# nomadkaraoke/python-audio-separator

Measured on AMD Instinct MI355X. Metric: audio-sec separated / wall-sec (RTF), UVR-MDX-NET 44.1kHz stereo, 1/2/4/8 GPU, higher is better.
Workload: dtype f32 (I/O and accumulators; matrix products on the 16-bit pipe from block-scaled two-part fp16 operands, 22-bit products -- see arithmetic; fp32-exact setting timed in arithmetic_ab)

## Files before the change

python-audio-separator_amd/csrc/asx.hip:

```cpp
#include <hip/hip_runtime.h>

#include <algorithm>
#include <atomic>
#include <cmath>
#include <cstdarg>
#include <cstdio>
#include <cstdlib>
#include <cstring>
#include <functional>
#include <map>
#include <string>
#include <mutex>
#include <vector>

#include "../../include/asx.h"
#include "knobs.h"
#include "resample_plan.h"
#include "flac_dec_plan.h"

static void grant_lds(const void *kernel, int bytes) {
  static std::mutex mu;
  static std::map<const void *, int> granted;
  std::lock_guard<std::mutex> lock(mu);
  int &g = granted[kernel];
// ... 35 lines not shown
#include "engine_mdx.h"

static int opt_nonneg(int32_t v) { return v < 0 ? 0 : (int)v; }
static int opt_onoff(int32_t v) { return v > 0 ? 1 : 0; }

static const struct EngineOption {
  const char *key;
  int asx_engine::*field;
  int EngineKnobs::*knob;
  int (*norm)(int32_t);
  const char *refusal = nullptr;
  int shipped = 0;
} kOptions[] = {
    {"winograd", &asx_engine::winograd, &EngineKnobs::winograd, opt_nonneg,
     "asx_set_option: winograd = %d names a superseded kernel generation that only an experimental build carries "
     "(python build.py --experimental); this library has 0 (direct kernel) and 3 (the default)", 3},
    {"winograd_stationary", &asx_engine::winos, &EngineKnobs::winos, opt_nonneg,
     "asx_set_option: the weight-stationary Winograd kernel (measured slower) is in experimental builds only (python build.py --experimental)"},
    {"winograd_bf16x6", &asx_engine::wino6, &EngineKnobs::wino6, opt_nonneg},
    {"gemm_bf16x6", &asx_engine::gemm_bf16x6, &EngineKnobs::gemm_bf16x6, opt_onoff},
    {"gemm_f16x3", &asx_engine::gemm_f16x3, &EngineKnobs::gemm_f16x3, opt_onoff},
    {"conv_direct_f16x3", &asx_engine::conv3h, &EngineKnobs::conv3h, opt_nonneg},
    {"conv_fuse_input", &asx_engine::conv_fuse_input, &EngineKnobs::conv_fuse_input, opt_onoff},
    {"conv3h_partial_scratch", &asx_engine::conv3h_ps, &EngineKnobs::conv3h_ps, opt_onoff},
    {"conv3h_walk", &asx_engine::conv3h_walk, &EngineKnobs::conv3h_walk, opt_onoff},
    {"conv3h_tiled", &asx_engine::conv3h_tiled, &EngineKnobs::conv3h_tiled, opt_onoff},
    {"conv_down_bf16x6", &asx_engine::down6, &EngineKnobs::down6, opt_onoff},
    {"conv_up_bf16x6", &asx_engine::up6, &EngineKnobs::up6, opt_onoff},
    {"gemm_pair_images", &asx_engine::pair_images, &EngineKnobs::pair_images, opt_onoff,
     "asx_set_option: gemm_pair_images = 1 needs an experimental build (python build.py --experimental): the pair-image reader measured no "
     "faster in the nets and is not in the default library"},
};

static const EngineOption *find_option(const char *fn, const char *key) {
  for (const EngineOption &o : kOptions)
    if (!strcmp(key, o.key)) return &o;
  set_err("%s: unknown option '%s'", fn, key);
  return nullptr;
}

extern "C" {

int asx_abi_version(void) { return ASX_ABI_VERSION; }
const char *asx_last_error(void) { return g_err; }

int asx_device_count(void) {
// ... 115 lines not shown
  }
  *out = e;
  return ASX_OK;
}

static void v3_destroy(V3Net *n);
static void rof_destroy(RofNet *n);
static void ht_destroy(HtNet *n);
static void hd_destroy(HdNet *n);
static void hd_drop_clones(asx_engine *e);
static void vr_destroy(VrNet *n);
static void ens_destroy(EnsCtx *c);
static void free_conv(ConvLayer &L) {
  L.w.release();
  L.b.release();
  L.wu.release();
  L.wu2.release();
  L.wu3.release();
  L.wus.release();
  L.wu6.release();
  L.wu6h.release();
  L.w3h.release();
  L.w1f.release();
  L.wd6.release();
  L.wup6.release();
  L.gn_w.release();
  L.gn_b.release();
}
static void free_tdf(TdfLayer &L) {
  L.w.release();
  L.bias.release();
  L.scale.release();
  L.shift.release();
  L.gn_w.release();
  L.gn_b.release();
}
static void free_block(Block &b) {
  for (auto &c : b.tfc) free_conv(c);
  free_tdf(b.tdf0);
  free_tdf(b.tdf1);
}

void asx_engine_destroy(asx_engine *e) {
  w3_flush(e);
  if (!e) return;
  (void)hipSetDevice(e->device);
// ... 2461 lines not shown
  BufGuard g{{&dw, &dp, &ds}};
  CHK(to_dev(dw, wave_host, (size_t)2 * n_samples));
  if (primary_host) CHK(dp.ensure((size_t)2 * n_out * 4));
  if (secondary_host) CHK(ds.ensure((size_t)2 * n_out * 4));
  CHK(vr_separate_dev(e, dw.f(), n_samples, params, primary_host ? dp.f() : nullptr, secondary_host ? ds.f() : nullptr, nullptr));
  if (primary_host) CHK(to_host(primary_host, dp, (size_t)2 * n_out));
  if (secondary_host) CHK(to_host(secondary_host, ds, (size_t)2 * n_out));
  return ASX_OK;
}

int asx_counter(const asx_engine *e, const char *name, int64_t *out) {
  REQUIRE(e && name && out, "asx_counter: null argument");
  const std::string nm(name);
  if (nm == "tdf3_launches") *out = (int64_t)g_tdf3_launches.load();
  else if (nm == "tdf3h_launches") *out = (int64_t)g_tdf3h_launches.load();
  else if (nm == "attn6_launches") *out = (int64_t)g_attn6_launches.load();
  else if (nm == "attn6h_launches") *out = (int64_t)g_attn6h_launches.load();
  else if (nm == "tdf3_gather_launches") *out = (int64_t)g_tdf3_gather_launches.load();
  else if (nm == "wino6_launches") *out = (int64_t)g_wino6_launches.load();
  else if (nm == "wino6h_launches") *out = (int64_t)g_wino6h_launches.load();
  else if (nm == "conv3h_launches") *out = (int64_t)g_conv3h_launches.load();
  else if (nm == "conv3h_fin_launches") *out = (int64_t)g_conv3h_fin_launches.load();
  else if (nm == "conv3h_tiled_launches") *out = (int64_t)g_conv3h_tiled_launches.load();
  else if (nm == "tdf3_pair_image_launches") *out = (int64_t)g_tdf3ps_launches.load();
  else if (nm == "down6_launches") *out = (int64_t)g_down6_launches.load();
  else if (nm == "up6_launches") *out = (int64_t)g_up6_launches.load();
  else if (nm == "hd_rounds") *out = (int64_t)g_hd_rounds.load();
  else if (nm == "vr_net_passes") *out = (int64_t)g_vr_net_passes.load();
  else if (nm == "v3_net_passes") *out = (int64_t)g_v3_net_passes.load();
  else if (nm == "rof_net_passes") *out = (int64_t)g_rof_net_passes.load();
  else if (nm == "flac_block_cycles") *out = (int64_t)e->flac_block_cycles;
  else if (nm == "flac_crc16_cycles") *out = (int64_t)e->flac_crc16_cycles;
  else {
    set_err("asx_counter: unknown counter '%s'", name);
    return ASX_ERR_INVALID;
  }
  return ASX_OK;
}

int asx_debug_trace(uint64_t *host, int64_t n_u64) {
  REQUIRE(host && n_u64 > 0 && n_u64 <= 4096 * 8, "asx_debug_trace: bad argument");
  HIPCHK(hipDeviceSynchronize());
  HIPCHK(hipMemcpyFromSymbol(host, HIP_SYMBOL(asx_dbg_trace), (size_t)n_u64 * 8));
  return ASX_OK;
}

// ... 258 lines not shown
```

python-audio-separator_amd/csrc/engine_core.h:

```cpp
#pragma once

static thread_local char g_err[512] = "";
static void set_err(const char *fmt, ...) {
  va_list ap;
  va_start(ap, fmt);
  vsnprintf(g_err, sizeof(g_err), fmt, ap);
  va_end(ap);
}
#define HIPCHK(x)                                                                       \
  do {                                                                                  \
    hipError_t e_ = (x);                                                                \
    if (e_ != hipSuccess) {                                                             \
      set_err("%s:%d %s -> %s", __FILE__, __LINE__, #x, hipGetErrorString(e_));         \
      return ASX_ERR_HIP;                                                               \
    }                                                                                   \
  } while (0)
#define CHK(x)                    \
  do {                            \
    int r_ = (x);                 \
    if (r_ != ASX_OK) return r_;  \
  } while (0)
#define REQUIRE(cond, ...)        \
  do {                            \
    if (!(cond)) {                \
// ... 56 lines not shown
  return to_host(out_host, dout, n_out);
}

enum ConvKind { CK_3X3 = 0, CK_DOWN = 1, CK_1X1 = 2, CK_UP = 3 };

struct ConvLayer {
  int kind = CK_3X3;
  int cin = 0, cout = 0;
  int nrep = 0, kc = 0, cg = 0, nci = 0;
  int relu = 1;
  DevBuf w, b;
  DevBuf wu;
  DevBuf wu2;
  DevBuf wu3;
  int wu_cg = 0, wu_nci = 0, wu3_nci = 0;
  DevBuf wus;
  int wus_ks = 0;
  DevBuf gn_w, gn_b;
  DevBuf wu6;
  int wu6_nci = 0;
  DevBuf wu6h;
  DevBuf w3h;
  DevBuf w1f;
  DevBuf wd6;
  int wd6_cg = 0, wd6_nst = 0, wd6_nrep = 3;
  DevBuf wup6;
  int wup6_cg = 0, wup6_nst = 0;
};

struct TdfLayer {
  int n = 0, k = 0, c = 0;
  bool has_bias = false;
  DevBuf w, bias, scale, shift;
  DevBuf gn_w, gn_b;
};

struct Block {
  std::vector<ConvLayer> tfc;
  TdfLayer tdf0, tdf1;
  int c = 0, t = 0, f = 0;
};

struct ProfRec {
  int cls;
  int nprod;
  hipEvent_t a, b;
// ... 79 lines not shown
  DevBuf flac_cycles;
  long long flac_block_cycles = 0, flac_crc16_cycles = 0;
  DevBuf flac_frames, flac_off;
  DevBuf flacdec_list, flacdec_slots, flacdec_accept;
  std::vector<flacdec::Accept> flacdec_accept_host;
  int64_t flacdec_n_samples = -1, flacdec_n_frames = 0;
  int32_t flacdec_channels = 0, flacdec_bps = 0, flacdec_max_bs = 0;
  size_t flacdec_slot_off = 0;
  std::vector<RsTable *> rs_tabs;
  std::mutex rs_mu;
  hipEvent_t div_ev = nullptr;
  hipStream_t div_stream = nullptr;
  std::vector<DevBuf> skip;
  int winograd = 3;
  int winos = 0;
  int gemm_bf16x6 = 1;
  int gemm_f16x3 = 1;
  int wino6 = 144;
  int conv3h = 144;
  int conv3h_ps = 1;
  int conv3h_walk = 1;
  int conv3h_tiled = 1;
  int conv_fuse_input = 1;
  int down6 = 1;
  int up6 = 1;
  int pair_images = 0;
  std::vector<W3Entry> w3;
  std::mutex w3_mu;
  bool prof = false;
  int prof_nprod = 0;
  std::vector<ProfRec> recs;
};

static int pick_batch(const asx_engine *e) { return e->cfg.max_batch > 0 ? e->cfg.max_batch : 64; }

#include "batching.h"

template <class F>
static int timed(asx_engine *e, int cls, double flops, double bytes, hipStream_t s, F &&launch) {
  if (!e->prof) {
    launch();
    HIPCHK(hipGetLastError());
    return ASX_OK;
  }
  ProfRec r;
  r.cls = cls;
// ... 65 lines not shown
```

python-audio-separator_amd/csrc/engine_mdx.h:

```cpp
#pragma once

template <class CFG>
static void launch_conv_t(const ConvArgs &a, int nblk, hipStream_t s) {
  grant_lds(&conv_mfma_kernel<CFG>, CFG::LDS_BYTES);
  hipLaunchKernelGGL(conv_mfma_kernel<CFG>, dim3(nblk), dim3(256), CFG::LDS_BYTES, s, a);
}

static int conv_tile_h(int kind) { return kind == CK_UP ? 4 : 8; }

static int pick_nrep_conv(int cout) {
  const int ct = (cout + 15) / 16;
  int best = 1, best_pad = 1 << 30;
  for (int n = 3; n >= 1; --n) {
    const int pad = ((ct + n - 1) / n) * n - ct;
    if (pad < best_pad) {
      best_pad = pad;
      best = n;
    }
  }
  return best;
}
static int pick_nrep_up(int cout) {
  const int ct = (cout + 15) / 16;
  if (knobs().up_nrep == 4 && (4 * ct) % 4 == 0) return 4;
// ... 134 lines not shown
        for (int c = 0; c < L.cin; ++c) {
          const float *g = &w[((size_t)co * L.cin + c) * 9];
          double t[4][3];
          for (int a = 0; a < 4; ++a)
            for (int j = 0; j < 3; ++j) t[a][j] = G[a][0] * g[0 * 3 + j] + G[a][1] * g[1 * 3 + j] + G[a][2] * g[2 * 3 + j];
          float *dst = &wus[(size_t)(co / 48) * per];
          for (int a = 0; a < 4; ++a)
            for (int bb = 0; bb < 4; ++bb) {
              const float u = (float)(t[a][0] * G[bb][0] + t[a][1] * G[bb][1] + t[a][2] * G[bb][2]);
              dst[L.wus_ks == 12 ? winos_u_index<12>(a, bb, c, co % 48) : winos_u_index<24>(a, bb, c, co % 48)] = u;
            }
        }
      CHK(L.wus.ensure(wus.size() * 4));
      HIPCHK(hipMemcpy(L.wus.p, wus.data(), wus.size() * 4, hipMemcpyHostToDevice));
    }
#endif
  }
  if (L.kind == CK_1X1 && L.cin == 4 && L.cout == Conv3hCfg::C) {
    std::vector<float> w1((size_t)Conv3hCfg::C * 5, 0.f);
    memcpy(w1.data(), w, (size_t)Conv3hCfg::C * 4 * 4);
    if (b) memcpy(w1.data() + Conv3hCfg::C * 4, b, (size_t)Conv3hCfg::C * 4);
    CHK(L.w1f.ensure(w1.size() * 4));
    HIPCHK(hipMemcpy(L.w1f.p, w1.data(), w1.size() * 4, hipMemcpyHostToDevice));
  }
  if (L.kind == CK_DOWN) {
    std::vector<uint32_t> w6;
    L.wd6_nrep = (knobs().down6_wide && L.cout % 96 == 0) ? 6 : 3;
    if (L.wd6_nrep == 6) down6_pack<6>(w, L.cout, L.cin, w6, &L.wd6_cg, &L.wd6_nst);
    else down6_pack<3>(w, L.cout, L.cin, w6, &L.wd6_cg, &L.wd6_nst);
    CHK(L.wd6.ensure(w6.size() * 4));
    HIPCHK(hipMemcpy(L.wd6.p, w6.data(), w6.size() * 4, hipMemcpyHostToDevice));
  }
  if (L.kind == CK_UP) {
    std::vector<uint32_t> w6;
    if (L.nrep == 6) up6_pack<6>(w, L.cout, L.cin, w6, &L.wup6_cg, &L.wup6_nst);
    else if (L.nrep == 4) up6_pack<4>(w, L.cout, L.cin, w6, &L.wup6_cg, &L.wup6_nst);
    else up6_pack<2>(w, L.cout, L.cin, w6, &L.wup6_cg, &L.wup6_nst);
    CHK(L.wup6.ensure(w6.size() * 4));
    HIPCHK(hipMemcpy(L.wup6.p, w6.data(), w6.size() * 4, hipMemcpyHostToDevice));
  }
  const int nb = (L.kind == CK_UP) ? CT * 16 : std::max(L.cg * NW, ((L.cout + 47) / 48) * 48);
  std::vector<float> bp(nb, 0.f);
  for (int i = 0; i < L.cout; ++i) bp[i] = b ? b[i] : 0.f;
  CHK(L.w.ensure(wp.size() * 4));
  CHK(L.b.ensure(bp.size() * 4));
  HIPCHK(hipMemcpy(L.w.p, wp.data(), wp.size() * 4, hipMemcpyHostToDevice));
// ... 645 lines not shown
  }
#endif
  launch_tdf3_abl<NREP, MREP, 0>(a, w3, s);
  return true;
}

static int tdf3_tile_form(const asx_engine *e, const TdfDmaArgs &d) {
  const int t128 = knobs().gemm_t128;
  const int small = knobs().tdf2_small;
  if (!tdf3_ok(e, d) || d.N <= 64) return 0;
  if (d.N <= 128) return 1;
  if ((small && d.K <= small) || d.prefer_small) return 1;
  const double rows = (double)((d.M + 127) / 128);
  auto cost = [&](int bn, double eff) {
    const double blocks = rows * (double)((d.N + bn - 1) / bn);
    return ceil(blocks / 512.0) * bn / eff;
  };
  const double eff128 = knobs().tdf3_eff128;
  const double e128 = (e->gemm_f16x3 > 0 && d.K <= 512 && !knobs().tdf3_eff128_set) ? 1.0 : eff128;
  const bool narrow3 = t128 == 2 || (t128 == 1 && cost(128, e128) < cost(192, 1.0));
  return narrow3 ? 2 : 3;
}

static bool tdf3h_will_run(asx_engine *e, const TdfDmaArgs &d, hipStream_t s) {
  const bool dbg = knobs().tdf3_abl_set || knobs().f16x3_n_set;
  if (dbg || e->gemm_f16x3 <= 0 || e->pair_images <= 0 || tdf3_tile_form(e, d) == 0) return false;
  return w3_image(e, d.w, d.N, d.K, s, 0, 1) != nullptr;
}
static int tdf3_tile_cols(const asx_engine *e, const TdfDmaArgs &d) { return tdf3_tile_form(e, d) == 3 ? 192 : 128; }
static void tdf3_set_xexp(TdfDmaArgs &d, const int *tab, int cols) {
  d.xexp = tab;
  d.xexp_gs = cols / 32;
  d.xexp_n = (d.K + cols - 1) / cols;
  d.xexp_inv = (65536 + d.xexp_gs - 1) / d.xexp_gs;
}

static void launch_tdf_dma_auto(asx_engine *e, const TdfDmaArgs &d, hipStream_t s) {
  const int t128 = knobs().gemm_t128;
  const bool v2 = tdf2_ok(d);
  const int small = knobs().tdf2_small;
  const int form = tdf3_tile_form(e, d);
  if (form == 1 && d.N > 128 && launch_tdf3<2, 4>(e, d, s)) return;
  if (v2 && ((small && d.K <= small) || d.prefer_small) && d.N > 128) return launch_tdf2<2, 4>(d, s);
  if (d.N > 128) {
    const double rows = (double)((d.M + 127) / 128);
    auto cost = [&](int bn, double eff) {
      const double blocks = rows * (double)((d.N + bn - 1) / bn);
      return ceil(blocks / 512.0) * bn / eff;
    };
    const bool narrow = t128 == 2 || (t128 == 1 && cost(128, 0.96) < cost(192, 1.0));
    if (form == 2 && launch_tdf3<2, 8>(e, d, s)) return;
    if (form == 3 && launch_tdf3<3, 8>(e, d, s)) return;
    if (narrow) v2 ? launch_tdf2<2, 8>(d, s) : launch_tdf_dma_t<2, 8>(d, s);
    else v2 ? launch_tdf2<3, 8>(d, s) : launch_tdf_dma_t<3, 8>(d, s);
  } else if (d.N > 64) {
    if (form == 1 && launch_tdf3<2, 4>(e, d, s)) return;
    v2 ? launch_tdf2<2, 4>(d, s) : launch_tdf_dma_t<2, 4>(d, s);
// ... 45 lines not shown
  TdfDmaArgs d;
  tdf_fill_args(e, L, x, res, y, M, T, relu, d);
  if (pair_out) {
    d.yexp = pair_out;
    d.yexp_n = (L.n + pair_cols - 1) / pair_cols;
  }
  if (pair_in) tdf3_set_xexp(d, pair_in, pair_cols);
  if ((pair_out || pair_in) && !dma) {
    set_err("tdf_launch: pair image on a layer the row-GEMM kernels cannot take");
    return ASX_ERR_STATE;
  }
  return timed(e, ASX_PROF_TDF, flops, bytes, s, [&]() {
    if (dma) {
      launch_tdf_dma_auto(e, d, s);
    } else {
      if (L.n > 128) launch_tdf_t<3, 8>(a, s);
      else if (L.n > 64) launch_tdf_t<2, 4>(a, s);
      else launch_tdf_t<1, 4>(a, s);
    }
  });
}

static int tdf_pair_launch(asx_engine *e, const TdfLayer &L0, const TdfLayer &L1, const float *x, float *H, int *HE, float *out, int64_t M, int T,
                           hipStream_t s) {
  int *pair_tab = nullptr;
  int pair_cols = 0;
  if (M > 0 && HE != nullptr) {
    TdfDmaArgs d0, d1;
    tdf_fill_args(e, L0, x, nullptr, H, M, T, 1, d0);
    tdf_fill_args(e, L1, H, x, out, M, T, 1, d1);
    const bool al = ((reinterpret_cast<uintptr_t>(x) | reinterpret_cast<uintptr_t>(H)) & 15) == 0 && !knobs().no_dma;
    if (al && L0.n % 32 == 0 && L0.k % 4 == 0 && L1.k % 4 == 0 && tdf3h_will_run(e, d0, s) && tdf3h_will_run(e, d1, s)) {
      pair_cols = tdf3_tile_cols(e, d0);
      pair_tab = HE;
    }
  }
  CHK(tdf_launch(e, L0, x, nullptr, H, M, T, s, 1, pair_tab, nullptr, pair_cols));
  return tdf_launch(e, L1, H, x, out, M, T, s, 1, nullptr, pair_tab, pair_cols);
}

static int tdf_pack(TdfLayer &L, int n, int k, int c, const float *w, const float *bias, const float *scale,
                    const float *shift) {
  L.n = n;
  L.k = k;
  L.c = c;
  L.has_bias = bias != nullptr;
  CHK(L.w.ensure((size_t)n * k * 4));
  HIPCHK(hipMemcpy(L.w.p, w, (size_t)n * k * 4, hipMemcpyHostToDevice));
  if (bias) {
    CHK(L.bias.ensure((size_t)n * 4));
    HIPCHK(hipMemcpy(L.bias.p, bias, (size_t)n * 4, hipMemcpyHostToDevice));
  }
  if (scale && shift) {
    CHK(L.scale.ensure((size_t)c * 4));
    CHK(L.shift.ensure((size_t)c * 4));
    HIPCHK(hipMemcpy(L.scale.p, scale, (size_t)c * 4, hipMemcpyHostToDevice));
    HIPCHK(hipMemcpy(L.shift.p, shift, (size_t)c * 4, hipMemcpyHostToDevice));
  }
  return ASX_OK;
}
// ... 115 lines not shown
      else hipLaunchKernelGGL(f3::istft3p_kernel<0>, dim3(ng, 2, B), dim3(256), f3::ISTFT3P_LDS_BYTES, s, f);
    }
    else
      hipLaunchKernelGGL(f3::istft3_kernel, dim3(ng, 2, B), dim3(256), f3::ISTFT3_LDS_BYTES, s, f);
    if (ng > 1) hipLaunchKernelGGL(f3::seam3_kernel, dim3(5, ng - 1, B * 2), dim3(256), 0, s, f);
  });
}

static int gn_launch(asx_engine *e, const float *x, int B, int C, int64_t P, const DevBuf &gw, const DevBuf &gb, const float *res,
                     const float *mul, float *y, hipStream_t s) {
  if (B <= 0) return ASX_OK;
  REQUIRE(C % 2 == 0 && gw.p && gb.p && e->gn_part.bytes >= (size_t)B * C * 16, "GroupNorm(2, %d): channels / workspace", C);
  double2 *part = reinterpret_cast<double2 *>(e->gn_part.p);
  const double bytes = 4.0 * (double)B * C * (double)P;
  CHK(timed(e, ASX_PROF_MISC, 0.0, bytes, s,
            [&]() { hipLaunchKernelGGL(gn_partial_kernel, dim3((unsigned)C, (unsigned)B), dim3(256), 0, s, x, C, P, part); }));
  const int nx = (int)std::max<int64_t>(1, std::min<int64_t>(32, (P / 4 + 1023) / 1024));
  return timed(e, ASX_PROF_MISC, 0.0, bytes * (2 + (res ? 1 : 0) + (mul ? 1 : 0)), s, [&]() {
    hipLaunchKernelGGL(gn_apply_kernel, dim3((unsigned)nx, (unsigned)C, (unsigned)B), dim3(256), 0, s, x, C, 2, P, part, gw.f(), gb.f(), 1e-5f, 1, res,
                       mul, y);
  });
}

static int block_forward(asx_engine *e, const Block &blk, float *&cur, float *dest, int B, hipStream_t s, const float *fin_x = nullptr) {
  auto next_free = [&](const float *a, const float *b) -> float * {
    for (int i = 0; i < 3; ++i)
      if (e->R[i].f() != a && e->R[i].f() != b) return e->R[i].f();
    return nullptr;
  };
  const bool gn = e->net.norm == 1;
  const int64_t plane = (int64_t)blk.t * blk.f;
  auto c3h = [&](size_t j, const float *xin) {
    const ConvLayer &L = blk.tfc[j];
    const bool dma = blk.f % 4 == 0 && (reinterpret_cast<uintptr_t>(xin) & 15) == 0 && !knobs().no_dma;
    return conv3h_takes(e, L, dma, nullptr, L.relu ? ACT_RELU : ACT_NONE, blk.t, blk.f, (int64_t)L.cout * plane, e->R[0].f()) && conv3h_tiled_ok(e, L, blk.t);
  };
  bool in_tiled = false;
  for (size_t j = 0; j < blk.tfc.size(); ++j) {
    float *out = next_free(cur, nullptr);
    ConvView v;
    if (j == 0 && fin_x) {
      v.fin = &e->first;
      v.fin_x = fin_x;
    }
    v.x_tiled = in_tiled;
    v.y_tiled = e->conv3h_tiled > 0 && !gn && j + 1 < blk.tfc.size() && (in_tiled || c3h(j, j == 0 && fin_x ? fin_x : cur)) && c3h(j + 1, out);
    in_tiled = v.y_tiled;
// ... 13 lines not shown
  if (bnk == 0) {
    float *out = dest ? dest : next_free(cur, nullptr);
    if (gn) {
      float *tmp = next_free(cur, out);
      CHK(tdf_launch(e, blk.tdf0, cur, nullptr, tmp, M, blk.t, s, 0));
      CHK(gn_launch(e, tmp, B, blk.c, plane, blk.tdf0.gn_w, blk.tdf0.gn_b, cur, nullptr, out, s));
    } else {
      CHK(tdf_launch(e, blk.tdf0, cur, cur, out, M, blk.t, s));
    }
    cur = out;
    return ASX_OK;
  }
  if (gn) {
    CHK(tdf_launch(e, blk.tdf0, cur, nullptr, e->H.f(), M, blk.t, s, 0));
    CHK(gn_launch(e, e->H.f(), B, blk.c, (int64_t)blk.t * (blk.f / bnk), blk.tdf0.gn_w, blk.tdf0.gn_b, nullptr, nullptr, e->H.f(), s));
    float *out = dest ? dest : next_free(cur, nullptr);
    float *tmp = dest ? next_free(cur, nullptr) : out;
    CHK(tdf_launch(e, blk.tdf1, e->H.f(), nullptr, tmp, M, blk.t, s, 0));
    CHK(gn_launch(e, tmp, B, blk.c, plane, blk.tdf1.gn_w, blk.tdf1.gn_b, cur, nullptr, out, s));
    cur = out;
    return ASX_OK;
  }
  float *out = dest ? dest : (knobs().tdf_inplace ? cur : next_free(cur, nullptr));
  CHK(tdf_pair_launch(e, blk.tdf0, blk.tdf1, cur, e->H.f(), reinterpret_cast<int *>(e->HE.p), out, M, blk.t, s));
  cur = out;
  return ASX_OK;
}

static int net_forward_dev(asx_engine *e, const float *spec_in, float *spec_out, int B, hipStream_t s) {
  if (!e->net_ready) {
    set_err("net weights not committed");
    return ASX_ERR_STATE;
  }
  const int T = e->net.dim_t, F = e->net.dim_f;
  const int n = e->net.num_blocks / 2;
  const bool gn = e->net.norm == 1;
  float *cur = e->R[0].f();
  const Block &blk0 = n > 0 ? e->enc[0] : e->mid;
  const bool fuse = e->conv_fuse_input > 0 && !gn && e->first.kind == CK_1X1 && e->first.cin == 4 && e->first.cout == Conv3hCfg::C && e->first.relu &&
                    e->first.w1f.p != nullptr && !blk0.tfc.empty() && blk0.tfc[0].cin == Conv3hCfg::C && blk0.tfc[0].cout == Conv3hCfg::C &&
                    conv3h_takes(e, blk0.tfc[0], F % 4 == 0 && (reinterpret_cast<uintptr_t>(spec_in) & 15) == 0 && !knobs().no_dma, nullptr,
                                 blk0.tfc[0].relu ? ACT_RELU : ACT_NONE, T, F, (int64_t)Conv3hCfg::C * T * F, e->R[1].f());
  if (!fuse) {
    CHK(conv_launch(e, e->first, spec_in, nullptr, cur, B, T, F, s));
    if (gn) CHK(gn_launch(e, cur, B, e->net.g, (int64_t)T * F, e->first.gn_w, e->first.gn_b, nullptr, nullptr, cur, s));
  }
  const float *fin_x = fuse ? spec_in : nullptr;
  for (int i = 0; i < n; ++i) {
    CHK(block_forward(e, e->enc[i], cur, e->skip[i].f(), B, s, i == 0 ? fin_x : nullptr));
    float *out = e->R[0].f();
    CHK(conv_launch(e, e->ds[i], cur, nullptr, out, B, e->enc[i].t, e->enc[i].f, s));
    if (gn)
      CHK(gn_launch(e, out, B, e->ds[i].cout, (int64_t)(e->enc[i].t / 2) * (e->enc[i].f / 2), e->ds[i].gn_w, e->ds[i].gn_b, nullptr, nullptr, out, s));
    cur = out;
  }
  CHK(block_forward(e, e->mid, cur, nullptr, B, s, n == 0 ? fin_x : nullptr));
  for (int i = 0; i < n; ++i) {
    const Block &blk = e->dec[i];
    float *out = nullptr;
    for (int r = 0; r < 3; ++r)
      if (e->R[r].f() != cur) {
        out = e->R[r].f();
        break;
      }
    CHK(conv_launch(e, e->us[i], cur, gn ? nullptr : e->skip[n - 1 - i].f(), out, B, blk.t / 2, blk.f / 2, s));
    if (gn)
      CHK(gn_launch(e, out, B, e->us[i].cout, (int64_t)blk.t * blk.f, e->us[i].gn_w, e->us[i].gn_b, nullptr, e->skip[n - 1 - i].f(), out, s));
    cur = out;
    CHK(block_forward(e, blk, cur, nullptr, B, s));
  }
  CHK(conv_launch(e, e->final_, cur, nullptr, spec_out, B, T, F, s));
  return ASX_OK;
}

static int net_walks_ensure(asx_engine *e, int Bn) {
  auto walks = [&](const Block &blk) -> int {
    for (const ConvLayer &L : blk.tfc) CHK(conv3h_walk_ensure(e, L, Bn, blk.t, blk.f));
    return ASX_OK;
  };
  for (const Block &blk : e->enc) CHK(walks(blk));
  CHK(walks(e->mid));
  for (const Block &blk : e->dec) CHK(walks(blk));
  return ASX_OK;
}

static int ensure_workspace(asx_engine *e, int Bchunks, bool need_net) {
  const int T = e->cfg.segment_size, Fq = e->cfg.dim_f;
  const int mult = (need_net && e->cfg.enable_denoise) ? 2 : 1;
  const size_t Bn = (size_t)Bchunks * mult;
  CHK(e->spec_in.ensure(Bn * 4 * T * Fq * 4));
  CHK(e->frames.ensure((size_t)Bchunks * 2 * T * e->cfg.n_fft * 4));
  if (need_net) {
    CHK(e->spec_out.ensure(Bn * 4 * T * Fq * 4));
    const size_t lvl0 = Bn * e->net.g * T * Fq * 4;
// ... 25 lines not shown
```

python-audio-separator_amd/csrc/kernels_gemm3.h:

```cpp
#pragma once
#include "kernels_net.h"

namespace asx {

typedef __bf16 bf16x8 __attribute__((ext_vector_type(8)));
typedef unsigned int u32x4 __attribute__((ext_vector_type(4)));

#define ASX_MFMA_BF16(a, b, c) __builtin_amdgcn_mfma_f32_16x16x32_bf16((a), (b), (c), 0, 0, 0)

__device__ __forceinline__ unsigned cvt_pk_bf16(float lo, float hi) {
  unsigned r;
  asm("v_cvt_pk_bf16_f32 %0, %1, %2" : "=v"(r) : "v"(lo), "v"(hi));
  return r;
}

__device__ __forceinline__ void split3_pair(float x0, float x1, unsigned &h, unsigned &m, unsigned &l) {
  h = cvt_pk_bf16(x0, x1);
  float r0 = __fsub_rn(x0, __uint_as_float(h << 16));
  float r1 = __fsub_rn(x1, __uint_as_float(h & 0xffff0000u));
  m = cvt_pk_bf16(r0, r1);
  r0 = __fsub_rn(r0, __uint_as_float(m << 16));
  r1 = __fsub_rn(r1, __uint_as_float(m & 0xffff0000u));
  l = cvt_pk_bf16(r0, r1);
}
// ... 152 lines not shown
    u32x4 h, l;
    split2h_oct(a, b, e, h, l);
    u32x4 *o = img + ((int64_t)(nt * nk + (it >> 6)) * 2) * 64 + (it & 63);
    o[0] = h;
    o[64] = l;
  }
  if (tid < 4) reinterpret_cast<int *>(img + (int64_t)ntiles * nk * 128)[nt * 4 + tid] = gexp[tid];
}

template <int V>
struct IntC {
  static constexpr int value = V;
};

struct RowGather {
  int O, I, KI, DO, DI, PO, PI, nch;
  int SO, SI, OR, IR;
  int cin;
  int ldc;
  int64_t x_bs;
};

constexpr int tdf3h_lds_bytes(int BM) { return 2 * 2 * BM * 64 + 16 * BM + 16; }
template <int NREP, int MREP, int ABL = 0, bool GATHER = false, bool H = false, bool PS = false, int NW = 4>
__global__ __launch_bounds__(64 * NW, NW == 4 ? 2 : 1) void tdf3_kernel(TdfDmaArgs a, const u32x4 *__restrict__ w3, RowGather gq) {
  static_assert(!PS || (H && !GATHER), "pair-image operands: fp16 x 3 arithmetic, plain row GEMM");
  static_assert(NW == 4 || (NW == 8 && MREP == 8 && !GATHER), "eight waves: 128-row tiles of the plain row GEMM");
  constexpr int NT = 64 * NW;
  constexpr int BM = 16 * MREP, BN = 16 * NREP * NW;
  constexpr int XC = BM * 4 / NT;
  constexpr int NP = H ? 2 : 3;
  constexpr int PART = BM * 64;
  constexpr int BUFB = NP * PART;
  static_assert(MREP % 4 == 0 && XC >= 1, "tile shape");
  extern __shared__ float lds_f[];
  char *lds = reinterpret_cast<char *>(lds_f);

  const int tid = threadIdx.x;
  const int lane = tid & 63;
  const int wave = __builtin_amdgcn_readfirstlane(tid >> 6);
  const int li = lane & 15, lk = lane >> 4;

  const int nbn = (a.N + BN - 1) / BN;
  int bg;
  int64_t bm_i;
  {
    const int nbm_i = (int)((a.M + BM - 1) / BM);
    const int xcd = blockIdx.x & 7, slot = blockIdx.x >> 3;
    if (a.tile_map == 2 && (nbn & 7) == 0 && (nbm_i & 7) == 0 && (((nbm_i >> 3) * (nbn >> 3)) & 7) == 0) {
      const int sid = (slot >> 6) * 8 + xcd, r = slot & 63, sc = nbn >> 3;
      bg = (sid % sc) * 8 + (r & 7);
      bm_i = (int64_t)(sid / sc) * 8 + (r >> 3);
    } else if (a.tile_map == 1) {
      const int lid = xcd_remap(blockIdx.x, gridDim.x);
      bg = lid % nbn;
      bm_i = lid / nbn;
    } else if ((gridDim.x & 7) == 0 && nbn >= 8 && (nbn & 7) == 0) {
      const int cx = nbn >> 3;
      bg = xcd * cx + slot % cx;
      bm_i = slot / cx;
    } else if ((gridDim.x & 7) == 0 && nbn < 8 && (8 % nbn) == 0 && nbm_i % (8 / nbn) == 0) {
      const int r = 8 / nbn;
      bg = xcd / r;
      bm_i = (int64_t)slot * r + (xcd % r);
    } else {
      const int lid = xcd_remap(blockIdx.x, gridDim.x);
      bg = lid % nbn;
      bm_i = lid / nbn;
    }
  }
  const int64_t m0 = bm_i * BM;
  const int n0 = bg * BN;
  const int64_t lda = a.lda ? a.lda : a.K, ldy = a.ldy ? a.ldy : a.N, ldr = a.ldr ? a.ldr : a.N;
  int nkx = a.K >> 5;
  if constexpr (GATHER) nkx = (a.K / gq.cin) * gq.nch;
  const int nk = (nkx + 1) & ~1;

  const int ntiles = (a.N + 15) >> 4;
  const u32x4 *wb[NREP];
#pragma unroll
  for (int n = 0; n < NREP; ++n) {
    int nt = (n0 >> 4) + wave * NREP + n;
    nt = nt < ntiles ? nt : ntiles - 1;
    wb[n] = w3 + (int64_t)nt * nk * (64 * NP) + lane;
  }
  u32x4 wr[2][NREP][NP];
  auto load_w = [&](auto par, int ks) {
    constexpr int P = decltype(par)::value;
#pragma unroll
    for (int n = 0; n < NREP; ++n)
#pragma unroll
      for (int p = 0; p < NP; ++p) wr[P][n][p] = wb[n][(int64_t)ks * (64 * NP) + p * 64];
  };

  auto hsw = [](int g) { return g == 0 ? 0 : (g == 1 ? 2 : (g == 2 ? 3 : 1)); };
  const float *xp[XC];
  int xw[XC];
  int po[XC], pi[XC];
#pragma unroll
  for (int i = 0; i < XC; ++i) {
    const int q = tid + NT * i;
    const int row = q >> 2, c = q & 3;
    int64_t r = m0 + row;
    if constexpr (GATHER) {
      const bool rok = r < a.M;
      r = rok ? r : a.M - 1;
      const int64_t img = (int64_t)gq.OR * gq.IR;
      const int64_t b = r / img;
      const int rem = (int)(r - b * img);
      const int oo = rem / gq.IR, jj = rem - oo * gq.IR;
      po[i] = oo * gq.SO;
      pi[i] = jj * gq.SI;
      xp[i] = a.x + b * gq.x_bs + ((int64_t)po[i] * gq.I + pi[i]) * gq.ldc + c * 8;
      if (!rok) po[i] = -(1 << 20);
    } else {
      r = r < a.M ? r : a.M - 1;
      xp[i] = a.x + r * lda + c * 8;
      po[i] = pi[i] = 0;
    }
    xw[i] = row * 64 + ((c ^ hsw((row >> 2) & 3)) << 4);
  }
  f32x4 xr[XC][2];
  const int *xe[XC];
  int ej[XC];
  auto load_x_sel = [&](int ks, int only) {
    const int kcs = ks < nkx ? ks : nkx - 1;
    if constexpr (GATHER) {
      const int tap = kcs / gq.nch, ch = kcs - tap * gq.nch;
      const int ky = tap / gq.KI, kx = tap - ky * gq.KI;
      const int dy = ky * gq.DO - gq.PO, dx = kx * gq.DI - gq.PI;
      const int off = (dy * gq.I + dx) * gq.ldc + ch * 32;
#pragma unroll
      for (int i = 0; i < XC; ++i) {
        if (only >= 0 && i != only) continue;
        const bool ok = (unsigned)(po[i] + dy) < (unsigned)gq.O && (unsigned)(pi[i] + dx) < (unsigned)gq.I &&
                        ch * 32 + (tid & 3) * 8 < gq.cin;
        const float *src = ok ? xp[i] + off : a.zeros;
        xr[i][0] = *reinterpret_cast<const f32x4 *>(src);
// ... 294 lines not shown
      const int oc = (c0 >> 1) + lk * 4;
      if (c0 < a.N && oc < a.glu_cout) {
        f32x4 bv = {0.f, 0.f, 0.f, 0.f}, bg = bv;
        if (a.bias != nullptr) {
          bv = *reinterpret_cast<const f32x4 *>(a.bias + c0 + lk * 4);
          bg = *reinterpret_cast<const f32x4 *>(a.bias + c0 + 16 + lk * 4);
        }
#pragma unroll
        for (int m = 0; m < MREP; ++m) {
          const int64_t row = m0 + m * 16 + li;
          if (row >= a.M) continue;
          const f32x4 v = acc[0][m] + bv, g4 = acc[1][m] + bg;
          f32x4 o4;
          o4.x = v.x * __builtin_amdgcn_rcpf(1.0f + __expf(-g4.x));
          o4.y = v.y * __builtin_amdgcn_rcpf(1.0f + __expf(-g4.y));
          o4.z = v.z * __builtin_amdgcn_rcpf(1.0f + __expf(-g4.z));
          o4.w = v.w * __builtin_amdgcn_rcpf(1.0f + __expf(-g4.w));
          *reinterpret_cast<f32x4 *>(a.y + row * ldy + oc) = o4;
        }
      }
      return;
    }
  }
#ifdef ASX_EXPERIMENTAL_KERNELS
  if constexpr (H && !GATHER) {
    if (a.yexp != nullptr) {
#pragma unroll
      for (int m = 0; m < MREP; ++m) {
        const int64_t row = m0 + m * 16 + li;
        const bool rok = row < a.M;
        const int c = rok ? (int)(((uint32_t)row / (uint32_t)a.T) % (uint32_t)a.C) : 0;
        const float sc = a.scale ? a.scale[c] : 1.f, sh = a.shift ? a.shift[c] : 0.f;
        const float rw = (rok && a.rscale) ? a.rscale[row] : 1.f;
        float mx = 0.f;
#pragma unroll
        for (int n = 0; n < NREP; ++n) {
          const int col = n0 + wave * 16 * NREP + n * 16 + lk * 4;
          const bool ok = rok && col < a.N;
          const f32x4 b4 = (ok && a.bias != nullptr) ? *reinterpret_cast<const f32x4 *>(a.bias + col) : (f32x4){0.f, 0.f, 0.f, 0.f};
          const f32x4 v = acc[n][m];
          f32x4 o;
          o.x = tdf_act(sc * __fmaf_rn(v.x, rw, b4.x) + sh, a.relu);
          o.y = tdf_act(sc * __fmaf_rn(v.y, rw, b4.y) + sh, a.relu);
          o.z = tdf_act(sc * __fmaf_rn(v.z, rw, b4.z) + sh, a.relu);
          o.w = tdf_act(sc * __fmaf_rn(v.w, rw, b4.w) + sh, a.relu);
          if (!ok) o = (f32x4){0.f, 0.f, 0.f, 0.f};
// ... 138 lines not shown
```

python-audio-separator_amd/csrc/kernels_net.h:

```cpp
#pragma once
#include <hip/hip_runtime.h>
#include <stdint.h>

namespace asx {

typedef float f32x4 __attribute__((ext_vector_type(4)));
typedef float f32x2 __attribute__((ext_vector_type(2)));

#define ASX_MFMA(a, b, c) __builtin_amdgcn_mfma_f32_16x16x4f32((a), (b), (c), 0, 0, 0)

__device__ __forceinline__ int xcd_remap(int bid, int nblk) {
  const int q = nblk >> 3, r = nblk & 7;
  const int xcd = bid & 7, slot = bid >> 3;
  const int base = (xcd < r) ? xcd * (q + 1) : r * (q + 1) + (xcd - r) * q;
  return base + slot;
}

enum { EPI_BIAS_ACT = 0, EPI_UP_MULSKIP = 1 };

template <int KH_, int KW_, int S_, int PAD_, int NREP_, int KC_, int RPW_, int EPI_>
struct ConvCfg {
  static constexpr int KH = KH_, KW = KW_, S = S_, PAD = PAD_, NREP = NREP_, KC = KC_, RPW = RPW_, EPI = EPI_;
  static constexpr int TH = 4 * RPW, TW = 64;
  static constexpr int IH = (TH - 1) * S + KH, IW = (TW - 1) * S + KW;
// ... 695 lines not shown
  conv_epilogue<CFG>(a, acc, b, cg, to0, fo0, wave, li, lk);
}

struct TdfDmaArgs {
  const float *x, *w, *bias, *scale, *shift, *res, *zeros;
  float *y;
  int64_t M;
  int N, K, C, T;
  int relu;
  int64_t lda, ldy, ldr;
  const float2 *rot_tab;
  int rot_cols, rot_half, rot_pos_mod;
  int64_t rot_pos_div;
  const float *rscale;
  int nt;
  int prefer_small;
  int tile_map;
  int glu_cout;
  const int *xexp;
  int xexp_n, xexp_gs;
  int xexp_inv;
  int *yexp;
  int yexp_n;
};

__device__ __forceinline__ f32x4 tdf_rot4(const TdfDmaArgs &a, f32x4 o, int64_t row, int col) {
  if (a.rot_tab == nullptr || col >= a.rot_cols) return o;
  const uint32_t pos = ((uint32_t)row / (uint32_t)a.rot_pos_div) % (uint32_t)a.rot_pos_mod;
  const int i = (col % (2 * a.rot_half)) >> 1;
  const float2 *t = a.rot_tab + (int64_t)pos * a.rot_half + i;
  const float2 c0 = t[0], c1 = t[1];
#ifdef ASX_ROT_PACKED
  f32x4 rp;
  rp.x = __fmaf_rn(o.x, c0.x, -__fmul_rn(o.y, c0.y));
  rp.y = __fmaf_rn(o.y, c0.x, __fmul_rn(o.x, c0.y));
  rp.z = __fmaf_rn(o.z, c1.x, -__fmul_rn(o.w, c1.y));
  rp.w = __fmaf_rn(o.w, c1.x, __fmul_rn(o.z, c1.y));
  return rp;
#endif
  float p0 = __fmul_rn(o.y, c0.y), p1 = __fmul_rn(o.x, c0.y), p2 = __fmul_rn(o.w, c1.y), p3 = __fmul_rn(o.z, c1.y);
  asm volatile("" : "+v"(p0));
  asm volatile("" : "+v"(p1));
  asm volatile("" : "+v"(p2));
  asm volatile("" : "+v"(p3));
  f32x4 r;
  r.x = __fmaf_rn(o.x, c0.x, -p0);
// ... 372 lines not shown
```

python-audio-separator_amd/csrc/knobs.h:

```cpp
#pragma once

#include <algorithm>
#include <climits>
#include <cstdint>
#include <cstdlib>

#ifndef ASX_TDF2_DEFAULT
#define ASX_TDF2_DEFAULT 1
#endif

constexpr int HD_MAX_GROUPS = 6;

namespace knob {
inline bool set(const char *name) { return getenv(name) != nullptr; }
inline int num(const char *name, int def) { return set(name) ? atoi(getenv(name)) : def; }
inline int64_t num64(const char *name, int64_t def) { return set(name) ? atoll(getenv(name)) : def; }
inline double real(const char *name, double def) { return set(name) ? atof(getenv(name)) : def; }
inline bool on_unless_0(const char *name) { return !(set(name) && atoi(getenv(name)) == 0); }
inline bool off_unless_nonzero(const char *name) { return set(name) && atoi(getenv(name)) != 0; }
inline int clamped(const char *name, int def, int lo, int hi = INT_MAX) { return set(name) ? std::max(lo, std::min(hi, atoi(getenv(name)))) : def; }
}

struct Knobs {
  int poison = knob::num("ASX_POISON", -1);
// ... 58 lines not shown
  bool rof_fuse = knob::on_unless_0("ASX_ROF_FUSE");
};

inline const Knobs &knobs() {
  static const Knobs k;
  return k;
}

struct EngineKnobs {
#ifdef ASX_EXPERIMENTAL_KERNELS
  int winograd = knob::clamped("ASX_WINOGRAD", 3, 0);
  int winos = knob::clamped("ASX_WINOS", 0, 0);
  int pair_images = knob::num("ASX_PAIR_IMAGES", 0);
#else
  int winograd = knob::num("ASX_WINOGRAD", 3) <= 0 ? 0 : 3;
  int winos = 0;
  int pair_images = 0;
#endif
  int gemm_bf16x6 = knob::num("ASX_GEMM_BF16X6", 1);
  int gemm_f16x3 = knob::num("ASX_GEMM_F16X3", 1);
  int wino6 = knob::clamped("ASX_WINO6", 144, 0);
  int conv3h = knob::clamped("ASX_CONV3H", 144, 0);
  int conv_fuse_input = 1;
  int conv3h_ps = 1;
  int conv3h_walk = 1;
  int conv3h_tiled = 1;
  int down6 = knob::num("ASX_DOWN6", 1);
  int up6 = knob::num("ASX_UP6", 1);
  bool fft3 = knob::on_unless_0("ASX_FFT3");
  bool fft3p = knob::on_unless_0("ASX_FFT3P");
};
```

Baseline: 1649.

## Fuse final 1x1 output conv into last TDF GEMM epilogue with channel-grouped tiles

Adds a channel-grouped tile mapping to the fp16x3 TDF GEMM kernel so that each 192-row tile covers all 48 channels for 4 frames. The epilogue then applies bias, scale/shift, ReLU and the residual, and reduces the 48→4 final 1x1 conv in registers using DPP quad shuffles. It writes the spectrogram output directly, skipping both the separate final conv launch and the round trip of the full 48-channel activation through memory. The path is gated by many shape, alignment and option checks and falls back to the old path otherwise. The channel-grouped row mapping may cost some locality in the GEMM input loads.

After: 1679, median of 6. 1.8% higher.

```diff
diff --git a/python-audio-separator_amd/csrc/asx.hip b/python-audio-separator_amd/csrc/asx.hip
--- a/python-audio-separator_amd/csrc/asx.hip
+++ b/python-audio-separator_amd/csrc/asx.hip
@@ -81,6 +81,7 @@
     {"gemm_f16x3", &asx_engine::gemm_f16x3, &EngineKnobs::gemm_f16x3, opt_onoff},
     {"conv_direct_f16x3", &asx_engine::conv3h, &EngineKnobs::conv3h, opt_nonneg},
     {"conv_fuse_input", &asx_engine::conv_fuse_input, &EngineKnobs::conv_fuse_input, opt_onoff},
+    {"tdf_fuse_output", &asx_engine::tdf_fuse_output, &EngineKnobs::tdf_fuse_output, opt_onoff},
     {"conv3h_partial_scratch", &asx_engine::conv3h_ps, &EngineKnobs::conv3h_ps, opt_onoff},
     {"conv3h_walk", &asx_engine::conv3h_walk, &EngineKnobs::conv3h_walk, opt_onoff},
     {"conv3h_tiled", &asx_engine::conv3h_tiled, &EngineKnobs::conv3h_tiled, opt_onoff},
@@ -242,6 +243,7 @@
   L.wu6h.release();
   L.w3h.release();
   L.w1f.release();
+  L.wof.release();
   L.wd6.release();
   L.wup6.release();
   L.gn_w.release();
@@ -2749,6 +2751,7 @@
   else if (nm == "conv3h_launches") *out = (int64_t)g_conv3h_launches.load();
   else if (nm == "conv3h_fin_launches") *out = (int64_t)g_conv3h_fin_launches.load();
   else if (nm == "conv3h_tiled_launches") *out = (int64_t)g_conv3h_tiled_launches.load();
+  else if (nm == "tdf_fused_output_launches") *out = (int64_t)g_tdf_fused_output_launches.load();
   else if (nm == "tdf3_pair_image_launches") *out = (int64_t)g_tdf3ps_launches.load();
   else if (nm == "down6_launches") *out = (int64_t)g_down6_launches.load();
   else if (nm == "up6_launches") *out = (int64_t)g_up6_launches.load();
diff --git a/python-audio-separator_amd/csrc/engine_core.h b/python-audio-separator_amd/csrc/engine_core.h
--- a/python-audio-separator_amd/csrc/engine_core.h
+++ b/python-audio-separator_amd/csrc/engine_core.h
@@ -102,6 +102,7 @@
   DevBuf wu6h;
   DevBuf w3h;
   DevBuf w1f;
+  DevBuf wof;
   DevBuf wd6;
   int wd6_cg = 0, wd6_nst = 0, wd6_nrep = 3;
   DevBuf wup6;
@@ -227,6 +228,7 @@
   int conv3h_walk = 1;
   int conv3h_tiled = 1;
   int conv_fuse_input = 1;
+  int tdf_fuse_output = 1;
   int down6 = 1;
   int up6 = 1;
   int pair_images = 0;
diff --git a/python-audio-separator_amd/csrc/engine_mdx.h b/python-audio-separator_amd/csrc/engine_mdx.h
--- a/python-audio-separator_amd/csrc/engine_mdx.h
+++ b/python-audio-separator_amd/csrc/engine_mdx.h
@@ -180,6 +180,14 @@
     if (b) memcpy(w1.data() + Conv3hCfg::C * 4, b, (size_t)Conv3hCfg::C * 4);
     CHK(L.w1f.ensure(w1.size() * 4));
     HIPCHK(hipMemcpy(L.w1f.p, w1.data(), w1.size() * 4, hipMemcpyHostToDevice));
+  }
+  if (L.kind == CK_1X1 && L.cin == TdfCgMap::C && L.cout == 4) {
+    std::vector<float> wo((size_t)TdfCgMap::C * 4 + 4, 0.f);
+    for (int oc = 0; oc < 4; ++oc)
+      for (int c = 0; c < TdfCgMap::C; ++c) wo[(size_t)c * 4 + oc] = w[(size_t)oc * TdfCgMap::C + c];
+    if (b) memcpy(wo.data() + TdfCgMap::C * 4, b, 4 * 4);
+    CHK(L.wof.ensure(wo.size() * 4));
+    HIPCHK(hipMemcpy(L.wof.p, wo.data(), wo.size() * 4, hipMemcpyHostToDevice));
   }
   if (L.kind == CK_DOWN) {
     std::vector<uint32_t> w6;
@@ -871,17 +879,49 @@
   return narrow3 ? 2 : 3;
 }
 
-static bool tdf3h_will_run(asx_engine *e, const TdfDmaArgs &d, hipStream_t s) {
+static bool tdf3h_takes(asx_engine *e, const TdfDmaArgs &d, hipStream_t s) {
   const bool dbg = knobs().tdf3_abl_set || knobs().f16x3_n_set;
-  if (dbg || e->gemm_f16x3 <= 0 || e->pair_images <= 0 || tdf3_tile_form(e, d) == 0) return false;
+  if (dbg || e->gemm_f16x3 <= 0 || tdf3_tile_form(e, d) == 0) return false;
   return w3_image(e, d.w, d.N, d.K, s, 0, 1) != nullptr;
 }
+static bool tdf3h_will_run(asx_engine *e, const TdfDmaArgs &d, hipStream_t s) { return e->pair_images > 0 && tdf3h_takes(e, d, s); }
 static int tdf3_tile_cols(const asx_engine *e, const TdfDmaArgs &d) { return tdf3_tile_form(e, d) == 3 ? 192 : 128; }
 static void tdf3_set_xexp(TdfDmaArgs &d, const int *tab, int cols) {
   d.xexp = tab;
   d.xexp_gs = cols / 32;
   d.xexp_n = (d.K + cols - 1) / cols;
   d.xexp_inv = (65536 + d.xexp_gs - 1) / d.xexp_gs;
+}
+
+static std::atomic<long long> g_tdf_fused_output_launches{0};
+struct TdfFusedOut {
+  const ConvLayer *fin;
+  float *out;
+  bool done;
+};
+static bool tdf_fused_output_ok(asx_engine *e, const TdfDmaArgs &d, const TdfFusedOut &fo, hipStream_t s) {
+  const ConvLayer &L = *fo.fin;
+  const int64_t ldr = d.ldr ? d.ldr : d.N;
+  return e->tdf_fuse_output > 0 && L.kind == CK_1X1 && L.cin == TdfCgMap::C && L.cout == 4 && !L.relu && L.wof.p != nullptr && L.gn_w.p == nullptr &&
+         d.C == TdfCgMap::C && d.T > 0 && d.T % TdfCgMap::TQ == 0 && d.N % TdfCgMap::BN == 0 && d.M > 0 && d.M % ((int64_t)TdfCgMap::C * d.T) == 0 &&
+         d.relu == 1 && d.res != nullptr && d.rscale == nullptr && d.rot_tab == nullptr && d.xexp == nullptr && d.yexp == nullptr && d.lda == 0 && d.ldy == 0 &&
+         (reinterpret_cast<uintptr_t>(fo.out) & 15) == 0 && (uint64_t)4 * (uint64_t)d.T * (uint64_t)ldr * 4 < (1ull << 31) &&
+         tdf3h_takes(e, d, s);
+}
+static void launch_tdf3_cg(asx_engine *e, const TdfDmaArgs &a0, const u32x4 *w3, hipStream_t s) {
+  constexpr int LDS_BYTES = tdf3h_lds_bytes(TdfCgMap::BM);
+  auto kern = tdf3_kernel<2, TdfCgMap::MREP, 0, false, true, false, 4, true>;
+  grant_lds(kern, LDS_BYTES);
+  TdfDmaArgs a = a0;
+  const int64_t nbm = a.M / TdfCgMap::BM;
+  const int nbn = a.N / TdfCgMap::BN;
+  const int map_env = knobs().tdf3_map;
+  a.tile_map = map_env >= 0 ? (nbn >= 8 ? map_env % 10 : map_env / 10) : (nbn < 8 ? 1 : 0);
+  e->prof_nprod = 3;
+  hipLaunchKernelGGL(kern, dim3((unsigned)(nbm * nbn)), dim3(256), LDS_BYTES, s, a, w3, RowGather{});
+  g_tdf3_launches.fetch_add(1);
+  g_tdf3h_launches.fetch_add(1);
+  g_tdf_fused_output_launches.fetch_add(1);
 }
 
 static void launch_tdf_dma_auto(asx_engine *e, const TdfDmaArgs &d, hipStream_t s) {
@@ -973,7 +1013,7 @@
 }
 
 static int tdf_pair_launch(asx_engine *e, const TdfLayer &L0, const TdfLayer &L1, const float *x, float *H, int *HE, float *out, int64_t M, int T,
-                           hipStream_t s) {
+                           hipStream_t s, TdfFusedOut *fo = nullptr) {
   int *pair_tab = nullptr;
   int pair_cols = 0;
   if (M > 0 && HE != nullptr) {
@@ -987,6 +1027,25 @@
     }
   }
   CHK(tdf_launch(e, L0, x, nullptr, H, M, T, s, 1, pair_tab, nullptr, pair_cols));
+  if (fo != nullptr && pair_tab == nullptr && M > 0 && L1.k % 4 == 0 && (reinterpret_cast<uintptr_t>(H) & 15) == 0 && !knobs().no_dma) {
+    TdfDmaArgs d;
+    tdf_fill_args(e, L1, H, x, out, M, T, 1, d);
+    if (tdf_fused_output_ok(e, d, *fo, s)) {
+      d.y = nullptr;
+      d.fo_w = fo->fin->wof.f();
+      d.fo_out = fo->out;
+      d.fo_bs = (int64_t)4 * T * L1.n;
+      const u32x4 *w3 = w3_image(e, d.w, d.N, d.K, s, 0, 1);
+      if (w3 != nullptr) {
+        const double bt = (double)M / TdfCgMap::C;
+        const double flops = 2.0 * (double)M * L1.n * L1.k + 2.0 * 4 * TdfCgMap::C * bt * L1.n;
+        const double bytes = 4.0 * ((double)M * L1.k + (double)M * L1.n + (double)L1.n * L1.k + 4.0 * bt * L1.n);
+        CHK(timed(e, ASX_PROF_TDF, flops, bytes, s, [&]() { launch_tdf3_cg(e, d, w3, s); }));
+        fo->done = true;
+        return ASX_OK;
+      }
+    }
+  }
   return tdf_launch(e, L1, H, x, out, M, T, s, 1, nullptr, pair_tab, pair_cols);
 }
 
@@ -1148,7 +1207,8 @@
   });
 }
 
-static int block_forward(asx_engine *e, const Block &blk, float *&cur, float *dest, int B, hipStream_t s, const float *fin_x = nullptr) {
+static int block_forward(asx_engine *e, const Block &blk, float *&cur, float *dest, int B, hipStream_t s, const float *fin_x = nullptr,
+                         TdfFusedOut *fo = nullptr) {
   auto next_free = [&](const float *a, const float *b) -> float * {
     for (int i = 0; i < 3; ++i)
       if (e->R[i].f() != a && e->R[i].f() != b) return e->R[i].f();
@@ -1208,7 +1268,7 @@
     return ASX_OK;
   }
   float *out = dest ? dest : (knobs().tdf_inplace ? cur : next_free(cur, nullptr));
-  CHK(tdf_pair_launch(e, blk.tdf0, blk.tdf1, cur, e->H.f(), reinterpret_cast<int *>(e->HE.p), out, M, blk.t, s));
+  CHK(tdf_pair_launch(e, blk.tdf0, blk.tdf1, cur, e->H.f(), reinterpret_cast<int *>(e->HE.p), out, M, blk.t, s, dest == nullptr ? fo : nullptr));
   cur = out;
   return ASX_OK;
 }
@@ -1240,7 +1300,10 @@
       CHK(gn_launch(e, out, B, e->ds[i].cout, (int64_t)(e->enc[i].t / 2) * (e->enc[i].f / 2), e->ds[i].gn_w, e->ds[i].gn_b, nullptr, nullptr, out, s));
     cur = out;
   }
-  CHK(block_forward(e, e->mid, cur, nullptr, B, s, n == 0 ? fin_x : nullptr));
+  TdfFusedOut fo{&e->final_, spec_out, false};
+  const Block &last = n > 0 ? e->dec[n - 1] : e->mid;
+  const bool try_fo = !gn && last.t == T && last.f == F;
+  CHK(block_forward(e, e->mid, cur, nullptr, B, s, n == 0 ? fin_x : nullptr, n == 0 && try_fo ? &fo : nullptr));
   for (int i = 0; i < n; ++i) {
     const Block &blk = e->dec[i];
     float *out = nullptr;
@@ -1253,9 +1316,9 @@
     if (gn)
       CHK(gn_launch(e, out, B, e->us[i].cout, (int64_t)blk.t * blk.f, e->us[i].gn_w, e->us[i].gn_b, nullptr, e->skip[n - 1 - i].f(), out, s));
     cur = out;
-    CHK(block_forward(e, blk, cur, nullptr, B, s));
-  }
-  CHK(conv_launch(e, e->final_, cur, nullptr, spec_out, B, T, F, s));
+    CHK(block_forward(e, blk, cur, nullptr, B, s, nullptr, i == n - 1 && try_fo ? &fo : nullptr));
+  }
+  if (!fo.done) CHK(conv_launch(e, e->final_, cur, nullptr, spec_out, B, T, F, s));
   return ASX_OK;
 }
 
diff --git a/python-audio-separator_amd/csrc/kernels_gemm3.h b/python-audio-separator_amd/csrc/kernels_gemm3.h
--- a/python-audio-separator_amd/csrc/kernels_gemm3.h
+++ b/python-audio-separator_amd/csrc/kernels_gemm3.h
@@ -198,10 +198,22 @@
 };
 
 constexpr int tdf3h_lds_bytes(int BM) { return 2 * 2 * BM * 64 + 16 * BM + 16; }
-template <int NREP, int MREP, int ABL = 0, bool GATHER = false, bool H = false, bool PS = false, int NW = 4>
+struct TdfCgMap {
+  static constexpr int C = 48, TQ = 4, MREP = 12, BM = C * TQ, BN = 128;
+  static constexpr int chan(int r) { return (r >> 4) * 4 + (r & 3); }
+  static constexpr int frame(int r) { return (r & 15) >> 2; }
+  static constexpr long long row_of(long long b, int tq, int r, int T) { return (b * C + chan(r)) * T + TQ * tq + frame(r); }
+  static constexpr long long row(long long bm_i, int r, int T) { return row_of(bm_i / (T / TQ), (int)(bm_i % (T / TQ)), r, T); }
+  static constexpr int out_oc(int lane) { return 2 * (lane & 1) + ((lane >> 1) & 1); }
+  static constexpr int out_frame(int lane) { return (lane & 15) >> 2; }
+  static constexpr int out_col(int wave, int lane, int j) { return wave * 32 + (j >> 2) * 16 + (lane >> 4) * 4 + (j & 3); }
+};
+
+template <int NREP, int MREP, int ABL = 0, bool GATHER = false, bool H = false, bool PS = false, int NW = 4, bool CG = false>
 __global__ __launch_bounds__(64 * NW, NW == 4 ? 2 : 1) void tdf3_kernel(TdfDmaArgs a, const u32x4 *__restrict__ w3, RowGather gq) {
   static_assert(!PS || (H && !GATHER), "pair-image operands: fp16 x 3 arithmetic, plain row GEMM");
   static_assert(NW == 4 || (NW == 8 && MREP == 8 && !GATHER), "eight waves: 128-row tiles of the plain row GEMM");
+  static_assert(!CG || (H && !GATHER && !PS && NW == 4 && NREP == 2 && MREP == TdfCgMap::MREP && ABL == 0), "channel-grouped tiles: 192 x 128, fp16 x 3");
   constexpr int NT = 64 * NW;
   constexpr int BM = 16 * MREP, BN = 16 * NREP * NW;
   constexpr int XC = BM * 4 / NT;
@@ -247,6 +259,8 @@
   }
   const int64_t m0 = bm_i * BM;
   const int n0 = bg * BN;
+  const int cg_b = CG ? (int)((uint32_t)bm_i / (uint32_t)(a.T >> 2)) : 0;
+  const int cg_tq = CG ? (int)((uint32_t)bm_i - (uint32_t)cg_b * (uint32_t)(a.T >> 2)) : 0;
   const int64_t lda = a.lda ? a.lda : a.K, ldy = a.ldy ? a.ldy : a.N, ldr = a.ldr ? a.ldr : a.N;
   int nkx = a.K >> 5;
   if constexpr (GATHER) nkx = (a.K / gq.cin) * gq.nch;
@@ -290,6 +304,7 @@
       xp[i] = a.x + b * gq.x_bs + ((int64_t)po[i] * gq.I + pi[i]) * gq.ldc + c * 8;
       if (!rok) po[i] = -(1 << 20);
     } else {
+      if constexpr (CG) r = TdfCgMap::row_of(cg_b, cg_tq, row, a.T);
       r = r < a.M ? r : a.M - 1;
       xp[i] = a.x + r * lda + c * 8;
       po[i] = pi[i] = 0;
@@ -630,6 +645,92 @@
       return;
     }
   }
+  if constexpr (CG) {
+    const int cl = li & 3, tl = li >> 2;
+    f32x4 bz[NREP];
+#pragma unroll
+    for (int n = 0; n < NREP; ++n)
+      bz[n] = (a.bias != nullptr) ? *reinterpret_cast<const f32x4 *>(a.bias + n0 + wave * 16 * NREP + n * 16 + lk * 4) : (f32x4){0.f, 0.f, 0.f, 0.f};
+    const uint32_t voff_r = (uint32_t)(((cl * a.T + tl) * (int)ldr + wave * 16 * NREP + lk * 4) * 4);
+    const char *rb0 = reinterpret_cast<const char *>(a.res) + ((((int64_t)cg_b * TdfCgMap::C) * a.T + TdfCgMap::TQ * cg_tq) * ldr + n0) * 4;
+    const int64_t rstep = (int64_t)4 * a.T * ldr * 4;
+    constexpr int RING = 4;
+    f32x4 rs[RING][NREP];
+    auto fetch = [&](int m) {
+      const char *rb = rb0 + m * rstep;
+#pragma unroll
+      for (int n = 0; n < NREP; ++n)
+        rs[m % RING][n] = (a.res == nullptr) ? (f32x4){0.f, 0.f, 0.f, 0.f}
+                          : ((a.nt & 2) ? __builtin_nontemporal_load(reinterpret_cast<const f32x4 *>(rb + voff_r + n * 64))
+                                        : *reinterpret_cast<const f32x4 *>(rb + voff_r + n * 64));
+    };
+#pragma unroll
+    for (int m = 0; m < RING; ++m) fetch(m);
+    const f32x4 *wq = reinterpret_cast<const f32x4 *>(a.fo_w) + cl;
+    float p[4][4 * NREP];
+#pragma unroll
+    for (int oc = 0; oc < 4; ++oc)
+#pragma unroll
+      for (int j = 0; j < 4 * NREP; ++j) p[oc][j] = 0.f;
+    f32x4 w4n = wq[0];
+    float scn = a.scale ? a.scale[cl] : 1.f, shn = a.shift ? a.shift[cl] : 0.f;
+#pragma unroll
+    for (int m = 0; m < MREP; ++m) {
+      const float sc = scn, sh = shn;
+      const float wv[4] = {w4n.x, w4n.y, w4n.z, w4n.w};
+      if (m + 1 < MREP) {
+        const int c = (m + 1) * 4 + cl;
+        w4n = wq[(m + 1) * 4];
+        scn = a.scale ? a.scale[c] : 1.f;
+        shn = a.shift ? a.shift[c] : 0.f;
+      }
+#pragma unroll
+      for (int n = 0; n < NREP; ++n) {
+        const f32x4 v = acc[n][m];
+        const f32x4 r = rs[m % RING][n];
+        float o[4];
+        o[0] = fmaxf(sc * (v.x + bz[n].x) + sh, 0.f) + r.x;
+        o[1] = fmaxf(sc * (v.y + bz[n].y) + sh, 0.f) + r.y;
+        o[2] = fmaxf(sc * (v.z + bz[n].z) + sh, 0.f) + r.z;
+        o[3] = fmaxf(sc * (v.w + bz[n].w) + sh, 0.f) + r.w;
+#pragma unroll
+        for (int oc = 0; oc < 4; ++oc) {
+#pragma unroll
+          for (int j = 0; j < 4; ++j) p[oc][n * 4 + j] = __fmaf_rn(wv[oc], o[j], p[oc][n * 4 + j]);
+          asm volatile("" : "+v"(p[oc][n * 4 + 0]), "+v"(p[oc][n * 4 + 1]), "+v"(p[oc][n * 4 + 2]), "+v"(p[oc][n * 4 + 3]));
+        }
+      }
+      if (m + RING < MREP) fetch(m + RING);
+      __builtin_amdgcn_sched_barrier(0);
+    }
+    auto quad_xor1 = [](float v) { return __int_as_float(__builtin_amdgcn_update_dpp(__float_as_int(v), __float_as_int(v), 0xB1, 0xf, 0xf, false)); };
+    auto quad_xor2 = [](float v) { return __int_as_float(__builtin_amdgcn_update_dpp(__float_as_int(v), __float_as_int(v), 0x4E, 0xf, 0xf, false)); };
+    const bool b0 = (cl & 1) != 0, b1 = (cl & 2) != 0;
+    float q[2][4 * NREP];
+#pragma unroll
+    for (int o2 = 0; o2 < 2; ++o2)
+#pragma unroll
+      for (int j = 0; j < 4 * NREP; ++j) {
+        const float keep = b0 ? p[2 + o2][j] : p[o2][j];
+        const float give = b0 ? p[o2][j] : p[2 + o2][j];
+        q[o2][j] = keep + quad_xor1(give);
+      }
+    const int oc = TdfCgMap::out_oc(lane);
+    const float bo = a.fo_w[4 * TdfCgMap::C + oc];
+    float *ob = a.fo_out + (int64_t)cg_b * a.fo_bs + ((int64_t)oc * a.T + TdfCgMap::TQ * cg_tq + tl) * a.N + n0 + wave * 16 * NREP + lk * 4;
+#pragma unroll
+    for (int n = 0; n < NREP; ++n) {
+      float r4[4];
+#pragma unroll
+      for (int j = 0; j < 4; ++j) {
+        const float keep = b1 ? q[1][n * 4 + j] : q[0][n * 4 + j];
+        const float give = b1 ? q[0][n * 4 + j] : q[1][n * 4 + j];
+        r4[j] = (keep + quad_xor2(give)) + bo;
+      }
+      *reinterpret_cast<f32x4 *>(ob + n * 16) = (f32x4){r4[0], r4[1], r4[2], r4[3]};
+    }
+    return;
+  }
 #ifdef ASX_EXPERIMENTAL_KERNELS
   if constexpr (H && !GATHER) {
     if (a.yexp != nullptr) {
diff --git a/python-audio-separator_amd/csrc/kernels_net.h b/python-audio-separator_amd/csrc/kernels_net.h
--- a/python-audio-separator_amd/csrc/kernels_net.h
+++ b/python-audio-separator_amd/csrc/kernels_net.h
@@ -741,6 +741,9 @@
   int xexp_inv;
   int *yexp;
   int yexp_n;
+  const float *fo_w;
+  float *fo_out;
+  int64_t fo_bs;
 };
 
 __device__ __forceinline__ f32x4 tdf_rot4(const TdfDmaArgs &a, f32x4 o, int64_t row, int col) {
diff --git a/python-audio-separator_amd/csrc/knobs.h b/python-audio-separator_amd/csrc/knobs.h
--- a/python-audio-separator_amd/csrc/knobs.h
+++ b/python-audio-separator_amd/csrc/knobs.h
@@ -104,6 +104,7 @@
   int wino6 = knob::clamped("ASX_WINO6", 144, 0);
   int conv3h = knob::clamped("ASX_CONV3H", 144, 0);
   int conv_fuse_input = 1;
+  int tdf_fuse_output = 1;
   int conv3h_ps = 1;
   int conv3h_walk = 1;
   int conv3h_tiled = 1;
```
